# CODEJIN/multi_speaker_tts

Hardware: AMD Instinct MI355X
Metric: mel-frames/sec (train step) at batch 32x(128 tok,800 mel) (higher is better)
Workload: dtype f32

## Files before the change

multi_speaker_tts_amd/csrc/gemm.hip:

```cpp
#include "common.h"
#include <type_traits>
#include <cmath>
#include <cstdlib>

namespace mstts {

typedef float f32x16 __attribute__((ext_vector_type(16)));

constexpr int BK = 32;
constexpr int BN = 128;

struct GemmArgs {
    const float* A; const float* B; float* C; const float* bias;
    int M, N, K;
    long lda, ldb, ldc;
    int win_T, win_C, win_pad, win_dil;
    int act, accumulate, split_k;
    long stride_a, stride_b, stride_c;
    float alpha;
    int k_per_split;
    int body, tail_s, tail_kps;
    int band;
};

// ... 143 lines not shown
        for (int i = 0; i < NV; ++i)
            *reinterpret_cast<float4*>(s + (kr + i * KR) * ldS + c4 * 4) = reg[i];
    }
};

template <int WM, int WN>
__device__ __forceinline__ void gemm_store_tile(const GemmArgs& g, const f32x16 (&acc)[WM][WN], float* __restrict__ C, int row0, int col0,
                                                int lane, bool with_bias, bool atomic) {
#pragma unroll
    for (int i = 0; i < WM; ++i)
#pragma unroll
        for (int j = 0; j < WN; ++j) {
            const int col = col0 + j * 32 + (lane & 31);
            if (col >= g.N) continue;
            const float bv = (g.bias != nullptr && with_bias) ? g.bias[col] : 0.f;
#pragma unroll
            for (int r = 0; r < 16; ++r) {
                const int row = row0 + i * 32 + (r & 3) + 8 * (r >> 2) + 4 * (lane >> 5);
                if (row >= g.M) continue;
                float v = g.alpha * acc[i][j][r] + bv;
                float* dst = C + (long)row * g.ldc + col;
                if (atomic) {
                    atomicAdd(dst, v);
                } else {
                    v = apply_act(v, g.act);
                    if (g.accumulate) v += *dst;
                    *dst = v;
                }
            }
        }
}

template <int BM, bool TA, bool TB, bool VEC>
__global__ __launch_bounds__(256) void gemm_kernel(GemmArgs g) {
    constexpr int LDA_S = TA ? BM + 4 : BM + 2, LDB_S = TB ? BN + 2 : BN + 4;
    constexpr int A_FLOATS = (BK * LDA_S + 3) / 4 * 4;
    __shared__ __attribute__((aligned(16))) float smem[A_FLOATS + BK * LDB_S];
    float* As = smem;
    float* Bs = smem + A_FLOATS;

    const int tiles_n = (g.N + BN - 1) / BN;
    int tile = blockIdx.x, piece = -1;
    if (tile < g.body) {
        const int nb = g.body, q = nb >> 3, r = nb & 7, xcd = tile & 7, idx = tile >> 3;
        if (nb >= 64) tile = xcd * q + (xcd < r ? xcd : r) + idx;
    } else {
        const int u = tile - g.body;
        tile = g.body + u / g.tail_s;
        piece = u % g.tail_s;
    }
    const int tile_m = tile / tiles_n, tile_n = tile % tiles_n;
    const int batch = blockIdx.z / g.split_k, split = blockIdx.z % g.split_k;
    const float* A = g.A + (long)batch * g.stride_a;
    const float* B = g.B + (long)batch * g.stride_b;
    float* C = g.C + (long)batch * g.stride_c;
    const int m0 = tile_m * BM, n0 = tile_n * BN;
    const int kbeg = piece >= 0 ? piece * g.tail_kps : split * g.k_per_split;
    const int kend = min(g.K, kbeg + (piece >= 0 ? g.tail_kps : g.k_per_split));

    using LA = typename std::conditional<TA, LoaderMC<BM, VEC>, LoaderKC<BM, VEC>>::type;
    using LB = typename std::conditional<TB, LoaderKC<BN, VEC>, LoaderMC<BN, VEC>>::type;
    LA la; LB lb;

    const int lane = threadIdx.x & 63, wave = threadIdx.x >> 6;
    constexpr int WM = (BM >= 64) ? 2 : 1;
    constexpr int WN = (BM == 128) ? 2 : 1;
    const int wm = (BM == 128) ? (wave >> 1) : 0;
    const int wn = (BM == 128) ? (wave & 1) : wave;
    const int wrow = wm * WM * 32, wcol = wn * WN * 32;

    f32x16 acc[WM][WN];
#pragma unroll
    for (int i = 0; i < WM; ++i)
#pragma unroll
        for (int j = 0; j < WN; ++j)
#pragma unroll
            for (int r = 0; r < 16; ++r) acc[i][j][r] = 0.f;

    auto load_a = [&](int k) {
        if constexpr (TA) la.load(k, kend, g.lda, g.win_T);
        else la.load(k, kend, g.win_T, g.win_C, g.win_pad, g.win_dil);
    };
    auto load_b = [&](int k) {
        if constexpr (TB) lb.load(k, kend, 0, 1, 0, 1);
        else lb.load(k, kend, g.ldb, 0);
    };
    la.prepare(A, g.lda, m0, kbeg, g.M, g.win_T, g.win_C, g.win_pad, g.win_dil);
    lb.prepare(B, g.ldb, n0, kbeg, g.N, 0, 1, 0, 1);
    if (kbeg < kend) {
        load_a(kbeg);
        load_b(kbeg);
    }
    for (int k0 = kbeg; k0 < kend; k0 += BK) {
        __syncthreads();
        la.store(As, LDA_S);
        lb.store(Bs, LDB_S);
        __syncthreads();
        if (k0 + BK < kend) {
            load_a(k0 + BK);
            load_b(k0 + BK);
        }
        const int kh = lane >> 5, l31 = lane & 31;
        float a[2][WM], b[2][WN];
#pragma unroll
        for (int i = 0; i < WM; ++i) a[0][i] = As[kh * LDA_S + wrow + i * 32 + l31];
#pragma unroll
        for (int j = 0; j < WN; ++j) b[0][j] = Bs[kh * LDB_S + wcol + j * 32 + l31];
#pragma unroll
        for (int kk = 0; kk < BK; kk += 2) {
            const int cur = (kk >> 1) & 1, nxt = cur ^ 1;
            if (kk + 2 < BK) {
#pragma unroll
                for (int i = 0; i < WM; ++i) a[nxt][i] = As[(kk + 2 + kh) * LDA_S + wrow + i * 32 + l31];
#pragma unroll
                for (int j = 0; j < WN; ++j) b[nxt][j] = Bs[(kk + 2 + kh) * LDB_S + wcol + j * 32 + l31];
            }
            __builtin_amdgcn_sched_barrier(0);
#pragma unroll
            for (int i = 0; i < WM; ++i)
#pragma unroll
                for (int j = 0; j < WN; ++j)
                    acc[i][j] = __builtin_amdgcn_mfma_f32_32x32x2f32(a[cur][i], b[cur][j], acc[i][j], 0, 0, 0);
            __builtin_amdgcn_sched_barrier(0);
        }
    }

    gemm_store_tile<WM, WN>(g, acc, C, m0 + wrow, n0 + wcol, lane, split == 0 && piece <= 0, g.split_k > 1 || piece >= 0);
}

__global__ void gemm_tail_act_kernel(float* __restrict__ C, long ldc, int N, long n, int act) {
    const long i = (long)blockIdx.x * 256 + threadIdx.x;
    if (i >= n) return;
    float* p = C + (i / N) * ldc + (i % N);
    *p = apply_act(*p, act);
}

template <int BM, bool TA, bool TB>
static void launch_gemm(const GemmArgs& g, bool vec, dim3 grid, hipStream_t st) {
    if (vec) hipLaunchKernelGGL((gemm_kernel<BM, TA, TB, true>), grid, dim3(256), 0, st, g);
    else     hipLaunchKernelGGL((gemm_kernel<BM, TA, TB, false>), grid, dim3(256), 0, st, g);
}

#include "gemm_split.inc"

}

using namespace mstts;

static int g_tail_split = 1;
extern "C" int mstts_gemm_tail_split(int32_t on) { g_tail_split = on != 0; return MSTTS_OK; }
static int g_split3 = 1;
extern "C" int mstts_gemm_split3(int32_t on) { g_split3 = on != 0; return MSTTS_OK; }
static int g_split_big = 1;
extern "C" int mstts_gemm_split_big(int32_t on) { g_split_big = on != 0; return MSTTS_OK; }
static int g_split_big_min = 160;
namespace mstts { void gemm_bf16_set_big_min(int n); }
extern "C" int mstts_gemm_big_min_workgroups(int32_t f32_split, int32_t bf16) {
    if (f32_split > 0) g_split_big_min = f32_split;
    gemm_bf16_set_big_min(bf16);
    return MSTTS_OK;
}
static thread_local int t_deterministic = 0;
extern "C" int mstts_gemm_deterministic(int32_t on) { t_deterministic = on != 0; return MSTTS_OK; }
namespace mstts { int gemm_deterministic_now() { return t_deterministic; } }

extern "C" int mstts_gemm_f32(const mstts_gemm_desc* d, mstts_stream_t stream) {
    MSTTS_REQUIRE(d != nullptr, MSTTS_ERR_SHAPE, "gemm: null descriptor");
    MSTTS_REQUIRE(d->M >= 0 && d->N >= 0 && d->K >= 0, MSTTS_ERR_SHAPE, "gemm: negative dims");
    if (d->M == 0 || d->N == 0) return MSTTS_OK;
    MSTTS_REQUIRE(d->A && d->B && d->C, MSTTS_ERR_SHAPE, "gemm: null operand");
    MSTTS_REQUIRE(d->M < (1LL << 31) && d->N < (1LL << 31) && d->K < (1LL << 31), MSTTS_ERR_SHAPE, "gemm: dims exceed int32");
    MSTTS_REQUIRE(d->lda >= 0 && d->ldb >= 0 && d->lda < (1 << 24) && d->ldb < (1 << 24), MSTTS_ERR_SHAPE,
                  "gemm: row strides must be below 2^24 elements (tile-relative offsets are 32-bit)");
    const int batch = d->batch > 0 ? (int)d->batch : 1;
    int split = d->split_k > 1 ? d->split_k : 1;
    MSTTS_REQUIRE(split == 1 || (d->act == MSTTS_ACT_NONE), MSTTS_ERR_SHAPE,
                  "gemm: split_k needs act=none (output must be pre-zeroed or accumulated into)");
    if (d->win_T > 0) {
        MSTTS_REQUIRE(d->win_C > 0 && d->lda == d->win_C, MSTTS_ERR_SHAPE, "gemm: window mode needs lda == win_C");
        MSTTS_REQUIRE(d->win_C % 4 == 0, MSTTS_ERR_SHAPE, "gemm: window mode needs win_C %% 4 == 0");
    }
    GemmArgs g;
    g.A = d->A; g.B = d->B; g.C = d->C; g.bias = d->bias;
    g.M = (int)d->M; g.N = (int)d->N; g.K = (int)d->K;
    g.lda = d->lda; g.ldb = d->ldb; g.ldc = d->ldc;
    g.win_T = d->win_T; g.win_C = d->win_C > 0 ? d->win_C : 1; g.win_pad = d->win_pad; g.win_dil = d->win_dil > 0 ? d->win_dil : 1;
    g.act = d->act; g.accumulate = d->accumulate; g.split_k = split;
    g.stride_a = d->stride_a; g.stride_b = d->stride_b; g.stride_c = d->stride_c;
    g.alpha = d->alpha;
    int kps = ((g.K + split - 1) / split + BK - 1) / BK * BK;
    if (kps < BK) kps = BK;
    g.k_per_split = kps;
    bool vec = aligned16(d->A) && aligned16(d->B) && (d->lda % 4 == 0) && (d->ldb % 4 == 0) &&
               (d->stride_a % 4 == 0) && (d->stride_b % 4 == 0);
    vec = vec && (d->trans_a ? (d->M % 4 == 0) : (d->K % 4 == 0));
    vec = vec && (d->trans_b ? (d->K % 4 == 0) : (d->N % 4 == 0));
    if (d->win_T > 0) vec = vec && (d->win_C % 4 == 0);
    const bool skinny = d->M <= 32;
    int bm = skinny ? 32 : 128, tail_s = 1, tail_rem = 0;
    const bool split3 = g_split3 && !skinny && d->K >= 160 && (d->win_T <= 0 || (d->win_T >= BK && d->win_C >= BK)) && gemm_split_lds_ready();
    if (!skinny) {
        const double t128 = (double)cdiv(d->M, 128) * cdiv(d->N, BN) * batch * split, t64 = (double)cdiv(d->M, 64) * cdiv(d->N, BN) * batch * split;
        const double e128 = t128 / (ceil(t128 / 256.0) * 256.0), e64 = t64 / (ceil(t64 / 256.0) * 256.0);
        if (e64 * 0.95 > e128 && !split3) bm = 64;
        if (g_tail_split && !t_deterministic && batch == 1 && split == 1 && (d->act == MSTTS_ACT_NONE || !d->accumulate)) {
            double best = (bm == 128 ? ceil(t128 / 256.0) : ceil(t64 / 256.0) * 0.54);
            const int ktiles = cdiv(d->K, BK);
            for (int cand = 128; cand >= (split3 ? 128 : 64); cand -= 64) {
                const long t = (long)cdiv(d->M, cand) * cdiv(d->N, BN);
                int rem = (int)(t % 256);
                if (d->act != MSTTS_ACT_NONE) rem = (int)(t - (t - rem) / cdiv(d->N, BN) * cdiv(d->N, BN));
                if (split3 && t <= 128) rem = (int)t;
                else if (t <= 256 || rem == 0 || rem > 128) continue;
                int s = 256 / rem;
                if (s > 16) s = 16;
                if (s > ktiles / 8) s = ktiles / 8;
                if (s < 2) continue;
                const double c = ((double)(t / 256) + 1.25 / s + 0.06) * (cand == 128 ? 1.0 : 0.54);
                if (c < best) { best = c; bm = cand; tail_s = s; tail_rem = rem; }
            }
        }
    }
    hipStream_t st = (hipStream_t)stream;
    {
        const long big_wgs = (long)cdiv(d->M, GSB_BM) * cdiv(d->N, GSB_BN) * batch * split;
        if (split3 && g_split_big && d->M >= 192 && d->N >= 192 && big_wgs >= g_split_big_min && d->lda < (1 << 22) && d->ldb < (1 << 22) &&
            (d->win_T <= 0 || (d->win_T >= GSB_BK && d->win_C >= GSB_BK)) && (d->act == MSTTS_ACT_NONE || split == 1) && gemm_split_big_ready()) {
            int kpsb = ((g.K + split - 1) / split + GSB_BK - 1) / GSB_BK * GSB_BK;
            if (kpsb < GSB_BK) kpsb = GSB_BK;
            g.k_per_split = kpsb;
            g.body = 0; g.tail_s = 1; g.tail_kps = kpsb; g.band = 0;
            dim3 gridb(cdiv(d->M, GSB_BM) * cdiv(d->N, GSB_BN), 1, batch * split);
            const bool ta_ = d->trans_a != 0, tb_ = d->trans_b != 0;
            if (!ta_ && !tb_) launch_gemm_split_big<false, false>(g, vec, gridb, st);
            else if (!ta_ && tb_) launch_gemm_split_big<false, true>(g, vec, gridb, st);
            else if (ta_ && !tb_) launch_gemm_split_big<true, false>(g, vec, gridb, st);
            else launch_gemm_split_big<true, true>(g, vec, gridb, st);
            MSTTS_CHECK_LAUNCH("gemm_f32 (split, 256 x 256 tile)");
            return MSTTS_OK;
        }
    }
    const int tiles = cdiv(d->M, bm) * cdiv(d->N, BN);
    g.body = tiles; g.tail_s = 1; g.tail_kps = kps;
    g.band = (split3 && tail_s == 1 && cdiv(d->N, BN) > 8) ? 8 : 0;
    if (tail_s > 1) {
        const int rem = tail_rem, tiles_n = cdiv(d->N, BN);
        g.body = tiles - rem; g.tail_s = tail_s;
        g.tail_kps = (cdiv(g.K, BK) + tail_s - 1) / tail_s * BK;
        if (!d->accumulate) {
            const long r0 = (long)(g.body / tiles_n) * bm;
            if (hipMemset2DAsync(d->C + r0 * d->ldc, (size_t)d->ldc * 4, 0, (size_t)d->N * 4, (size_t)(d->M - r0), st) != hipSuccess)
                MSTTS_REQUIRE(false, MSTTS_ERR_LAUNCH, "gemm: clearing the tail tiles failed");
        }
    }
    dim3 grid(g.body + (tiles - g.body) * g.tail_s, 1, batch * split);
    const bool ta = d->trans_a != 0, tb = d->trans_b != 0;
    if (split3) {
        if (!ta && !tb) launch_gemm_split<false, false>(g, vec, grid, st);
        else if (!ta && tb) launch_gemm_split<false, true>(g, vec, grid, st);
        else if (ta && !tb) launch_gemm_split<true, false>(g, vec, grid, st);
        else launch_gemm_split<true, true>(g, vec, grid, st);
    } else if (skinny) {
        if (!ta && !tb) launch_gemm<32, false, false>(g, vec, grid, st);
        else if (!ta && tb) launch_gemm<32, false, true>(g, vec, grid, st);
        else if (ta && !tb) launch_gemm<32, true, false>(g, vec, grid, st);
        else launch_gemm<32, true, true>(g, vec, grid, st);
    } else if (bm == 64) {
        if (!ta && !tb) launch_gemm<64, false, false>(g, vec, grid, st);
        else if (!ta && tb) launch_gemm<64, false, true>(g, vec, grid, st);
        else if (ta && !tb) launch_gemm<64, true, false>(g, vec, grid, st);
        else launch_gemm<64, true, true>(g, vec, grid, st);
    } else {
        if (!ta && !tb) launch_gemm<128, false, false>(g, vec, grid, st);
        else if (!ta && tb) launch_gemm<128, false, true>(g, vec, grid, st);
        else if (ta && !tb) launch_gemm<128, true, false>(g, vec, grid, st);
        else launch_gemm<128, true, true>(g, vec, grid, st);
    }
    MSTTS_CHECK_LAUNCH("gemm_f32");
    if (tail_s > 1 && d->act != MSTTS_ACT_NONE) {
        const long r0 = (long)(g.body / cdiv(d->N, BN)) * bm;
        const long n = (d->M - r0) * d->N;
        hipLaunchKernelGGL(gemm_tail_act_kernel, dim3((unsigned)cdiv(n, 256)), dim3(256), 0, st, d->C + r0 * d->ldc, d->ldc, (int)d->N, n, d->act);
        MSTTS_CHECK_LAUNCH("gemm_f32 tail activation");
    }
    return MSTTS_OK;
}
```

multi_speaker_tts_amd/csrc/gemm_split.inc:

```

typedef __bf16 gs_bf16x8 __attribute__((ext_vector_type(8)));
typedef __bf16 gs_bf16x4 __attribute__((ext_vector_type(4)));
constexpr int GS_BM = 128, GS_LD = 40;
constexpr int GS_PLANE = 128 * GS_LD;

struct Split3 { gs_bf16x4 hi, mid, lo; };
__device__ __forceinline__ uint32_t gs_cvt_pk(float a, float b) {
    uint32_t r;
    asm("v_cvt_pk_bf16_f32 %0, %1, %2" : "=v"(r) : "v"(a), "v"(b));
    return r;
}
__device__ __forceinline__ float gs_sub(float a, uint32_t b_bits) {
    float r;
    asm("v_sub_f32 %0, %1, %2" : "=v"(r) : "v"(a), "v"(b_bits));
    return r;
}
__device__ __forceinline__ void gs_split2(float x0, float x1, uint32_t& hi, uint32_t& mid, uint32_t& lo) {
    hi = gs_cvt_pk(x0, x1);
    x0 = gs_sub(x0, hi << 16); x1 = gs_sub(x1, hi & 0xffff0000u);
    mid = gs_cvt_pk(x0, x1);
    x0 = gs_sub(x0, mid << 16); x1 = gs_sub(x1, mid & 0xffff0000u);
    lo = gs_cvt_pk(x0, x1);
}
__device__ __forceinline__ Split3 gs_split4(float a, float b, float c, float d) {
// ... 200 lines not shown
        using LA = typename std::conditional<TA, GsLoaderMC<VEC, WIN>, GsLoaderKC<VEC, WIN>>::type;
        using LB = typename std::conditional<TB, GsLoaderKC<VEC, false>, GsLoaderMC<VEC, false>>::type;
        if (wave < 8) {
            const int tid = threadIdx.x - 256;
            LA la;
            la.prepare(tid, g.A + (long)batch * g.stride_a, g.lda, m0, kbeg, g.M, g.win_T, g.win_C, g.win_pad, g.win_dil);
            gs_produce([&](float4 (&r)[4], int k) {
                           if constexpr (TA) la.load(tid, r, k, kend, g.lda, g.win_T);
                           else la.load(tid, r, k, kend, g.win_T, g.win_C, g.win_pad, g.win_dil);
                       },
                       [&](const float4 (&r)[4], __bf16* dst) { la.store(tid, r, dst); }, gs_lds, kbeg, nt2);
        } else {
            const int tid = threadIdx.x - 512;
            LB lb;
            lb.prepare(tid, g.B + (long)batch * g.stride_b, g.ldb, n0, kbeg, g.N, 0, 1, 0, 1);
            gs_produce([&](float4 (&r)[4], int k) {
                           if constexpr (TB) lb.load(tid, r, k, kend, 0, 1, 0, 1);
                           else lb.load(tid, r, k, kend, g.ldb, 0);
                       },
                       [&](const float4 (&r)[4], __bf16* dst) { lb.store(tid, r, dst); }, gs_lds + 3 * GS_PLANE, kbeg, nt2);
        }
        return;
    }

    float* C = g.C + (long)batch * g.stride_c;
    const int lane = threadIdx.x & 63;
    const int wrow = (wave >> 1) * 64, wcol = (wave & 1) * 64;
    const int l31 = lane & 31, kg = lane >> 5;

    f32x16 acc[2][2];
#pragma unroll
    for (int i = 0; i < 2; ++i)
#pragma unroll
        for (int j = 0; j < 2; ++j)
#pragma unroll
            for (int r = 0; r < 16; ++r) acc[i][j][r] = 0.f;

    const int aoff = (wrow + l31) * GS_LD + kg * 8, boff = 3 * GS_PLANE + (wcol + l31) * GS_LD + kg * 8;
    gs_bf16x8 fa[2][2][3], fb[2][2][3];
    auto frags = [&](int set, const __bf16* buf, int ks) {
#pragma unroll
        for (int p = 0; p < 3; ++p) {
#pragma unroll
            for (int i = 0; i < 2; ++i) fa[set][i][p] = *reinterpret_cast<const gs_bf16x8*>(buf + aoff + p * GS_PLANE + i * 32 * GS_LD + ks * 16);
#pragma unroll
            for (int j = 0; j < 2; ++j) fb[set][j][p] = *reinterpret_cast<const gs_bf16x8*>(buf + boff + p * GS_PLANE + j * 32 * GS_LD + ks * 16);
        }
    };
    auto products = [&](int set) {
#pragma unroll
        for (int tt = 0; tt < GS_NPROD; ++tt) {
            const int pa = (tt == 0) ? 0 : (tt == 1) ? 1 : (tt == 2) ? 0 : (tt == 3) ? 1 : (tt == 4) ? 2 : 0;
            const int pb = (tt == 0) ? 0 : (tt == 1) ? 0 : (tt == 2) ? 1 : (tt == 3) ? 1 : (tt == 4) ? 0 : 2;
#pragma unroll
            for (int i = 0; i < 2; ++i)
#pragma unroll
                for (int j = 0; j < 2; ++j)
                    acc[i][j] = __builtin_amdgcn_mfma_f32_32x32x16_bf16(fa[set][i][pa], fb[set][j][pb], acc[i][j], 0, 0, 0);
        }
    };
    GS_BAR(0);
    frags(0, gs_lds, 0);
    for (int t = 0; t < nt2; ++t) {
        const __bf16* buf = gs_lds + (t & 1) * GS_BUF;
        frags(1, buf, 1);
        __builtin_amdgcn_sched_barrier(0);
        products(0);
        __builtin_amdgcn_sched_barrier(0);
        GS_BAR(0);
        frags(0, gs_lds + ((t + 1) & 1) * GS_BUF, 0);
        __builtin_amdgcn_sched_barrier(0);
        products(1);
        __builtin_amdgcn_sched_barrier(0);
    }
#ifdef GS_STAMP
    if (stamp && (threadIdx.x & 63) == 0) { unsigned long long* o = (unsigned long long*)g.bias; o[0] = acc_wait; o[1] = __builtin_readcyclecounter() - t_begin; o[2] = nt2; o[3] = wall_clock64() - w_begin; }
    if (stamp) return;
#endif
    gemm_store_tile<2, 2>(g, acc, C, m0 + wrow, n0 + wcol, lane, split == 0 && piece <= 0, g.split_k > 1 || piece >= 0);
}

constexpr int GSB_BM = 256, GSB_BN = 256, GSB_BK = 16, GSB_LD = 24, GSB_THREADS = 512;
constexpr int GSB_PLANE = 256 * GSB_LD;
constexpr int GSB_BUF = 6 * GSB_PLANE;
constexpr size_t GSB_LDS_BYTES = 2 * GSB_BUF * sizeof(__bf16);
__device__ __forceinline__ void gsb_put(__bf16* __restrict__ p, const Split3& s) {
    *reinterpret_cast<gs_bf16x4*>(p) = s.hi;
    *reinterpret_cast<gs_bf16x4*>(p + GSB_PLANE) = s.mid;
    *reinterpret_cast<gs_bf16x4*>(p + 2 * GSB_PLANE) = s.lo;
}
template <bool VEC, bool WIN>
struct GsbLoaderKC {
    static constexpr int NV = 2;
    const float* ubase;
    unsigned voff[2], rmask;
    int t_row[2], tap, kc, ld_;
    __device__ __forceinline__ bool mine(int) const { return true; }
    __device__ __forceinline__ void prepare(int tid, const float* __restrict__ base, long ld, int row0, int k0, int rows, int wT, int wC, int wpad, int wdil) {
        const int k4 = tid & 3, r = tid >> 2;
        rmask = 0; ld_ = (int)ld;
#pragma unroll
        for (int i = 0; i < 2; ++i) {
            const int row = row0 + r + i * 128;
            if (row < rows) rmask |= 1u << i;
            voff[i] = (unsigned)((r + i * 128) * (int)ld) + (WIN ? 0u : (unsigned)(k4 * 4));
            if (WIN) t_row[i] = row % wT;
        }
        if (WIN) {
            const int k = k0 + k4 * 4;
            tap = k / wC; kc = k - tap * wC;
            ubase = base + ((long)row0 - (long)wpad * wdil) * ld;
        } else {
            ubase = base + (long)row0 * ld + k0;
        }
    }
    __device__ __forceinline__ void load(int tid, float4 (&reg)[4], int k0, int kmax, long, int wT, int wC, int wpad, int wdil) {
        const int k4 = tid & 3;
        const int k = k0 + k4 * 4;
        const bool kok = k < kmax;
        const int sh = WIN ? (tap - wpad) * wdil : 0;
        const unsigned wadd = WIN ? (unsigned)(tap * wdil * ld_ + kc) : 0u;
#pragma unroll
        for (int i = 0; i < 2; ++i) {
            float4 v = make_float4(0.f, 0.f, 0.f, 0.f);
            bool ok = kok && ((rmask >> i) & 1u);
            if (WIN) {
                const int t = t_row[i] + sh;
                ok = ok && t >= 0 && t < wT;
            }
            if (VEC) {
                v = gemm_ld4(ok ? ubase + (voff[i] + wadd) : gemm_zero16);
            } else if (ok) {
                const float* p = ubase + (voff[i] + wadd);
                v.x = p[0];
                if (k + 1 < kmax) v.y = p[1];
                if (k + 2 < kmax) v.z = p[2];
                if (k + 3 < kmax) v.w = p[3];
            }
            reg[i] = v;
        }
        if (WIN) {
            kc += GSB_BK;
            const bool wrap = kc >= wC;
            kc -= wrap ? wC : 0; tap += wrap ? 1 : 0;
        } else {
            ubase += GSB_BK;
        }
    }
    __device__ __forceinline__ void store(int tid, const float4 (&reg)[4], __bf16* __restrict__ s) const {
        const int k4 = tid & 3, r = tid >> 2;
#pragma unroll
        for (int i = 0; i < 2; ++i) gsb_put(s + (r + i * 128) * GSB_LD + k4 * 4, gs_split4(reg[i].x, reg[i].y, reg[i].z, reg[i].w));
    }
};
template <bool VEC, bool WIN, int HALF>
struct GsbLoaderMC {
    const float* ubase;
    unsigned voff[4];
    int sh, t_k[4], cols_left;
    __device__ __forceinline__ bool mine(int tid) const { return (tid >> 8) == HALF; }
    __device__ __forceinline__ void prepare(int tid, const float* __restrict__ base, long ld, int col0, int k0, int cols, int wT, int wC, int wpad, int wdil) {
        const int u = tid & 255, kq = u & 3, c4 = u >> 2;
        const int col = col0 + c4 * 4;
        cols_left = cols - col;
        if (WIN) {
            const int tp = col / wC, cm = col - tp * wC;
            sh = (tp - wpad) * wdil;
#pragma unroll
            for (int i = 0; i < 4; ++i) {
                t_k[i] = (k0 + kq * 4 + i) % wT;
                voff[i] = (unsigned)((kq * 4 + i + tp * wdil) * (int)ld + cm);
            }
            ubase = base + ((long)k0 - (long)wpad * wdil) * ld;
        } else {
            sh = 0;
#pragma unroll
            for (int i = 0; i < 4; ++i) voff[i] = (unsigned)((kq * 4 + i) * (int)ld + c4 * 4);
            ubase = base + (long)k0 * ld + col0;
        }
    }
    __device__ __forceinline__ void load(int tid, float4 (&reg)[4], int k0, int kmax, long ld, int wT, int, int, int) {
        const int kq = tid & 3;
#pragma unroll
        for (int i = 0; i < 4; ++i) {
            const int k = k0 + kq * 4 + i;
            float4 v = make_float4(0.f, 0.f, 0.f, 0.f);
            bool ok = k < kmax && cols_left > 0;
            if (WIN) {
                const int t = t_k[i] + sh;
                ok = ok && t >= 0 && t < wT;
                t_k[i] += GSB_BK;
                t_k[i] -= (t_k[i] >= wT) ? wT : 0;
            }
            if (VEC) {
                v = gemm_ld4(ok ? ubase + voff[i] : gemm_zero16);
            } else if (ok) {
                const float* p = ubase + voff[i];
                v.x = p[0];
                if (cols_left > 1) v.y = p[1];
                if (cols_left > 2) v.z = p[2];
                if (cols_left > 3) v.w = p[3];
            }
            reg[i] = v;
        }
        ubase += GSB_BK * ld;
    }
    __device__ __forceinline__ void store(int tid, const float4 (&reg)[4], __bf16* __restrict__ s) const {
        const int u = tid & 255, kq = u & 3, c4 = u >> 2;
        __bf16* p = s + (c4 * 4) * GSB_LD + kq * 4;
        gsb_put(p, gs_split4(reg[0].x, reg[1].x, reg[2].x, reg[3].x));
        gsb_put(p + GSB_LD, gs_split4(reg[0].y, reg[1].y, reg[2].y, reg[3].y));
        gsb_put(p + 2 * GSB_LD, gs_split4(reg[0].z, reg[1].z, reg[2].z, reg[3].z));
        gsb_put(p + 3 * GSB_LD, gs_split4(reg[0].w, reg[1].w, reg[2].w, reg[3].w));
    }
};

template <bool TA, bool TB, bool VEC, bool WIN>
__global__ __launch_bounds__(GSB_THREADS) void gemm_split_big_kernel(GemmArgs g) {
    extern __shared__ __attribute__((aligned(16))) __bf16 gs_lds[];
    const int tiles_n = (g.N + GSB_BN - 1) / GSB_BN;
    int tile = blockIdx.x;
    {
        const int nb = gridDim.x, q = nb >> 3, r = nb & 7, xcd = tile & 7, idx = tile >> 3;
        if (nb >= 64) tile = xcd * q + (xcd < r ? xcd : r) + idx;
    }
    const int tile_m = tile / tiles_n, tile_n = tile % tiles_n;
    const int batch = blockIdx.z / g.split_k, split = blockIdx.z % g.split_k;
    float* C = g.C + (long)batch * g.stride_c;
    const int m0 = tile_m * GSB_BM, n0 = tile_n * GSB_BN;
    const int kbeg = split * g.k_per_split;
    const int kend = min(g.K, kbeg + g.k_per_split);
    const int nt = kend > kbeg ? (kend - kbeg + GSB_BK - 1) / GSB_BK : 0;
    const int tid = threadIdx.x, lane = tid & 63, wave = __builtin_amdgcn_readfirstlane(tid >> 6);
    const int wrow = (wave >> 2) * 128, wcol = (wave & 3) * 64;
    const int l31 = lane & 31, kg = lane >> 5;

    using LA = typename std::conditional<TA, GsbLoaderMC<VEC, WIN, 0>, GsbLoaderKC<VEC, WIN>>::type;
    using LB = typename std::conditional<TB, GsbLoaderKC<VEC, false>, GsbLoaderMC<VEC, false, 1>>::type;
    LA la; LB lb;
    const bool a_mine = la.mine(tid), b_mine = lb.mine(tid);
    if (a_mine) la.prepare(tid, g.A + (long)batch * g.stride_a, g.lda, m0, kbeg, g.M, g.win_T, g.win_C, g.win_pad, g.win_dil);
    if (b_mine) lb.prepare(tid, g.B + (long)batch * g.stride_b, g.ldb, n0, kbeg, g.N, 0, 1, 0, 1);
    float4 ra[4], rb[4];
    auto load = [&](int k) {
        if (a_mine) la.load(tid, ra, k, kend, g.lda, g.win_T, g.win_C, g.win_pad, g.win_dil);
        if (b_mine) lb.load(tid, rb, k, kend, g.ldb, 0, 1, 0, 1);
    };
    auto store = [&](int buf) {
        if (a_mine) la.store(tid, ra, gs_lds + buf * GSB_BUF);
        if (b_mine) lb.store(tid, rb, gs_lds + buf * GSB_BUF + 3 * GSB_PLANE);
    };

    f32x16 acc[4][2];
#pragma unroll
    for (int i = 0; i < 4; ++i)
#pragma unroll
        for (int j = 0; j < 2; ++j)
#pragma unroll
            for (int r = 0; r < 16; ++r) acc[i][j][r] = 0.f;

    const int aoff = (wrow + l31) * GSB_LD + kg * 8, boff = 3 * GSB_PLANE + (wcol + l31) * GSB_LD + kg * 8;
    gs_bf16x8 fb[2][3], fa0[4], fa1[4];
    auto ldA = [&](gs_bf16x8 (&f)[4], const __bf16* buf, int p) {
#pragma unroll
        for (int i = 0; i < 4; ++i) f[i] = *reinterpret_cast<const gs_bf16x8*>(buf + aoff + p * GSB_PLANE + i * 32 * GSB_LD);
    };
    auto ldB = [&](const __bf16* buf) {
#pragma unroll
        for (int p = 0; p < 3; ++p)
#pragma unroll
            for (int j = 0; j < 2; ++j) fb[j][p] = *reinterpret_cast<const gs_bf16x8*>(buf + boff + p * GSB_PLANE + j * 32 * GSB_LD);
    };
    auto mm = [&](const gs_bf16x8 (&f)[4], int pb) {
#pragma unroll
        for (int i = 0; i < 4; ++i)
#pragma unroll
            for (int j = 0; j < 2; ++j)
                acc[i][j] = __builtin_amdgcn_mfma_f32_32x32x16_bf16(f[i], fb[j][pb], acc[i][j], 0, 0, 0);
    };

    if (nt > 0) {
        load(kbeg);
        store(0);
        load(kbeg + GSB_BK);
        gs_barrier();
        for (int t = 0; t < nt; ++t) {
            const __bf16* buf = gs_lds + (t & 1) * GSB_BUF;
            ldB(buf); ldA(fa0, buf, 0); ldA(fa1, buf, 1);
            mm(fa0, 0); mm(fa0, 1); mm(fa0, 2);
            ldA(fa0, buf, 2);
            store((t + 1) & 1);
            load(kbeg + (t + 2) * GSB_BK);
            mm(fa1, 0); mm(fa1, 1);
            mm(fa0, 0);
            gs_barrier();
        }
    }
    gemm_store_tile<4, 2>(g, acc, C, m0 + wrow, n0 + wcol, lane, split == 0, g.split_k > 1);
}

static int gemm_split_big_ready() {
    static int memo[64];
    int dev = 0;
    if (hipGetDevice(&dev) != hipSuccess || dev < 0 || dev >= 64) return 0;
    if (!memo[dev]) {
        bool ok = true;
#define GSB_ATTR1(TA_, TB_, V_, W_) ok = ok && hipFuncSetAttribute((const void*)gemm_split_big_kernel<TA_, TB_, V_, W_>, hipFuncAttributeMaxDynamicSharedMemorySize, (int)GSB_LDS_BYTES) == hipSuccess
#define GSB_ATTR(TA_, TB_) GSB_ATTR1(TA_, TB_, true, true); GSB_ATTR1(TA_, TB_, true, false); GSB_ATTR1(TA_, TB_, false, true); GSB_ATTR1(TA_, TB_, false, false)
        GSB_ATTR(false, false); GSB_ATTR(false, true); GSB_ATTR(true, false); GSB_ATTR(true, true);
#undef GSB_ATTR
#undef GSB_ATTR1
        if (!ok) (void)hipGetLastError();
        memo[dev] = ok ? 2 : 1;
    }
    return memo[dev] == 2;
}

template <bool TA, bool TB>
static void launch_gemm_split_big(const GemmArgs& g, bool vec, dim3 grid, hipStream_t st) {
    const bool win = g.win_T > 0;
    if (vec && win)  hipLaunchKernelGGL((gemm_split_big_kernel<TA, TB, true, true>), grid, dim3(GSB_THREADS), GSB_LDS_BYTES, st, g);
    else if (vec)    hipLaunchKernelGGL((gemm_split_big_kernel<TA, TB, true, false>), grid, dim3(GSB_THREADS), GSB_LDS_BYTES, st, g);
    else if (win)    hipLaunchKernelGGL((gemm_split_big_kernel<TA, TB, false, true>), grid, dim3(GSB_THREADS), GSB_LDS_BYTES, st, g);
    else             hipLaunchKernelGGL((gemm_split_big_kernel<TA, TB, false, false>), grid, dim3(GSB_THREADS), GSB_LDS_BYTES, st, g);
}

static int gemm_split_lds_ready() {
    static int memo[64];
    int dev = 0;
    if (hipGetDevice(&dev) != hipSuccess || dev < 0 || dev >= 64) return 0;
    if (!memo[dev]) {
        bool ok = true;
#define GS_ATTR1(TA_, TB_, V_, W_) ok = ok && hipFuncSetAttribute((const void*)gemm_split_kernel<TA_, TB_, V_, W_>, hipFuncAttributeMaxDynamicSharedMemorySize, (int)GS_LDS_BYTES) == hipSuccess
#define GS_ATTR(TA_, TB_) GS_ATTR1(TA_, TB_, true, true); GS_ATTR1(TA_, TB_, true, false); GS_ATTR1(TA_, TB_, false, true); GS_ATTR1(TA_, TB_, false, false)
        GS_ATTR(false, false); GS_ATTR(false, true); GS_ATTR(true, false); GS_ATTR(true, true);
#undef GS_ATTR
#undef GS_ATTR1
        if (!ok) (void)hipGetLastError();
        memo[dev] = ok ? 2 : 1;
    }
    return memo[dev] == 2;
}

template <bool TA, bool TB>
static void launch_gemm_split(const GemmArgs& g, bool vec, dim3 grid, hipStream_t st) {
    const bool win = g.win_T > 0;
    if (vec && win)  hipLaunchKernelGGL((gemm_split_kernel<TA, TB, true, true>), grid, dim3(GS_THREADS), GS_LDS_BYTES, st, g);
    else if (vec)    hipLaunchKernelGGL((gemm_split_kernel<TA, TB, true, false>), grid, dim3(GS_THREADS), GS_LDS_BYTES, st, g);
    else if (win)    hipLaunchKernelGGL((gemm_split_kernel<TA, TB, false, true>), grid, dim3(GS_THREADS), GS_LDS_BYTES, st, g);
    else             hipLaunchKernelGGL((gemm_split_kernel<TA, TB, false, false>), grid, dim3(GS_THREADS), GS_LDS_BYTES, st, g);
}
```

multi_speaker_tts_amd/lib.py:

```python
from __future__ import annotations

import ctypes as C
import os

import torch

_HERE = os.path.dirname(os.path.abspath(__file__))
LIB_PATH = os.path.join(_HERE, "libmstts_hip.so")

ACT_NONE, ACT_RELU, ACT_TANH, ACT_SIGMOID = 0, 1, 2, 3

vp, i64, i32, f32, u64, u32 = C.c_void_p, C.c_int64, C.c_int32, C.c_float, C.c_uint64, C.c_uint32


class GemmDesc(C.Structure):
    _fields_ = [("A", vp), ("B", vp), ("C", vp), ("bias", vp),
                ("M", i64), ("N", i64), ("K", i64), ("lda", i64), ("ldb", i64), ("ldc", i64),
                ("trans_a", i32), ("trans_b", i32), ("win_T", i32), ("win_C", i32), ("win_pad", i32),
                ("act", i32), ("accumulate", i32), ("split_k", i32),
                ("batch", i64), ("stride_a", i64), ("stride_b", i64), ("stride_c", i64), ("alpha", f32), ("win_dil", i32)]


class LstmPointFwd(C.Structure):
    _fields_ = [("B", i64), ("H", i64), ("gates_h", vp), ("gates_parts", i32), ("gates_pstride", i64), ("xw", vp), ("xw_sb", i64), ("xw_st", i64), ("bias", vp),
# ... 141 lines not shown
    "mstts_lsa_proj_pack_floats": (i64, []),
    "mstts_lsa_proj_pack": (i32, [vp, i64, i64, i64, vp, vp]),
    "mstts_lsa_step_qp_ws_bytes": (i64, [i64, i64]),
    "mstts_lsa_step_prenet_supported": (i32, [i64, i64]),
    "mstts_lsa_step_fwd_qp": (i32, [P(LsaConst), vp, i64, vp, i64, vp, vp, vp, i64, i64, vp, vp, vp, vp, vp, vp, i64, vp, i64, P(CellPackedDst),
                                    P(LsaPrenet), vp, C.c_uint32, i32, vp]),
    "mstts_lsa_step_fwd_q": (i32, [P(LsaConst), vp, i64, vp, i64, i32, vp, vp, vp, vp, vp, i64, vp, i64, P(CellPackedDst), vp, C.c_uint32, i32, vp]),
    "mstts_lsa_step_fwd_selftest": (i32, [P(LsaConst), vp, i32, i64, vp, vp, vp, vp, vp, i64, vp, C.c_uint32, i32, vp]),
    "mstts_lsa_dalign_bwd": (i32, [P(LsaConst), vp, i64, vp, i64, i32, i64, vp, vp, vp, vp, vp]),
    "mstts_lsa_denergy_bwd": (i32, [P(LsaConst), vp, vp, vp, vp, vp, vp, vp, vp]),
    "mstts_lsa_param_bwd": (i32, [P(LsaConst), i64, vp, vp, vp, vp, vp, vp, vp, vp, vp]),
    "mstts_lsa_param_bwd_ws_floats": (i64, [i64, i64, i64]),
    "mstts_lsa_fold_location": (i32, [vp, vp, vp, vp, vp, i64, i64, i64, vp]),
    "mstts_lsa_filter_by_unit": (i32, [vp, vp, i64, i64, vp]),
    "mstts_lsa_unfold_location_grad": (i32, [vp, vp, vp, vp, vp, vp, vp, vp, i64, i64, i64, vp]),
    "mstts_tts_loss_fwd_bwd": (i32, [vp, vp, vp, vp, vp, i64, i64, i64, i32, f32, vp, vp, vp, vp, vp]),
    "mstts_l2_loss_acc": (i32, [vp, vp, i64, vp, vp]),
    "mstts_shift_frames": (i32, [vp, vp, i64, i64, i64, vp]),
    "mstts_unpack_proj": (i32, [vp, i64, vp, vp, i64, i64, i64, vp]),
    "mstts_pack_dproj": (i32, [vp, vp, vp, i64, i64, i64, i64, vp]),
    "mstts_speaker_tile": (i32, [vp, vp, vp, i64, i64, i64, i64, i64, vp]),
    "mstts_conv_kernel_flip": (i32, [vp, vp, i64, i64, i64, vp]),
    "mstts_transpose01": (i32, [vp, vp, i64, i64, i64, vp]),
    "mstts_speaker_finalize": (i32, [vp, vp, i64, i64, i64, i64, vp]),
    "mstts_adam_tf": (i32, [vp, vp, vp, vp, vp, f32, f32, f32, f32, f32, f32, i64, vp]),
    "mstts_stft_mel": (i32, [vp, i64, f32, vp, vp, i32, i32, i32, i32, f32, vp, vp, i64, vp]),
    "mstts_stft_mel_ws_floats": (i64, [i64, i32, i64]),
    "mstts_stft_fft_supported": (i32, [i32, i32]),
    "mstts_stft_fft": (i32, [vp, vp, vp, i32, f32, vp, vp, vp, vp, i32, i32, i32, i32, f32, f32, vp, vp, i64, vp, vp, f32, i32, vp]),
    "mstts_fold_rows": (i32, [vp, vp, i64, i64, i64, i64, vp]),
    "mstts_decoder_bf16_splits": (i32, [i64, i64, i64, P(i32)]),
    "mstts_skinny_bf16_fwd_splits": (i32, [i64, i64]),
    "mstts_skinny_bf16_bwd_splits": (i32, [i64, i64]),
    "mstts_pack_bf16_fwd": (i32, [vp, i64, vp, i64, i64, i32, vp]),
    "mstts_pack_bf16_bwd": (i32, [vp, i64, vp, i64, i64, i32, vp]),
    "mstts_skinny_fwd_bf16": (i32, [vp, i64, vp, vp, i64, i64, i64, i64, i32, vp]),
    "mstts_skinny_bwd_bf16": (i32, [vp, i64, vp, vp, i64, i64, i64, i64, i32, vp]),
    "mstts_ge2e_ws_floats": (i64, [i64, i64, i64]),
    "mstts_ge2e_loss_fwd_bwd": (i32, [vp, i64, i64, i64, i64, vp, vp, vp, i64, vp, vp]),
    "mstts_wg_overlap_add": (i32, [vp, vp, vp, i64, i64, i64, i64, i64, vp]),
    "mstts_wg_gate": (i32, [vp, i64, vp, i64, i64, vp]),
    "mstts_wg_gate_add": (i32, [vp, i64, vp, vp, i64, i64, vp]),
    "mstts_wg_res_skip": (i32, [vp, vp, vp, vp, i64, i64, i32, i32, vp]),
    "mstts_wg_coupling_inv": (i32, [vp, vp, vp, vp, f32, vp, i64, i64, i64, vp]),
    "mstts_philox_normal": (i32, [vp, i64, u64, u32, f32, vp]),
    "mstts_wg_weight_norm_fwd": (i32, [vp, i64, i64, vp]),
    "mstts_wg_weight_norm_bwd": (i32, [vp, i64, i64, vp]),
    "mstts_wg_coupling_fwd": (i32, [vp, vp, vp, vp, i64, i64, i64, vp, i64, i64, vp]),
    "mstts_wg_coupling_bwd": (i32, [vp, vp, vp, i64, i64, i64, vp, f32, vp, vp, i64, i64, vp]),
    "mstts_wg_inv1x1_logdet": (i32, [vp, vp, vp, i64, f32, vp, vp]),
    "mstts_wg_gate_bwd": (i32, [vp, i64, vp, vp, vp, i64, i64, i64, vp]),
    "mstts_wg_res_skip_bwd": (i32, [vp, vp, vp, vp, i64, i64, i32, vp]),
    "mstts_wg_overlap_add_bwd": (i32, [vp, vp, i64, i64, i64, i64, i64, i64, vp]),
    "mstts_wg_bias_fold": (i32, [vp, vp, vp, i64, i64, vp]),
    "mstts_adam_tf_clip": (i32, [vp, vp, vp, vp, vp, f32, f32, f32, f32, f32, f32, i64, vp]),
    "mstts_lstm_seq_fwd": (i32, [P(LstmSeqFwd), vp]),
    "mstts_lstm_seq_bwd": (i32, [P(LstmSeqBwd), vp]),
    "mstts_lstm_seq_fwd_pair": (i32, [P(LstmSeqFwd), P(LstmSeqFwd), vp]),
    "mstts_lstm_seq_bwd_pair": (i32, [P(LstmSeqBwd), P(LstmSeqBwd), vp]),
    "mstts_persist_lstm_supported": (i32, [i64, i64]),
    "mstts_persist_lstm_pack_floats": (i64, []),
    "mstts_persist_lstm_ws_bytes": (i64, []),
    "mstts_persist_lstm_pack": (i32, [vp, i64, vp, vp, vp]),
    "mstts_persist_lstm_supported_n": (i32, [i64, i64, i32]),
    "mstts_persist_lstm_fwd_supported_n": (i32, [i64, i64, i32]),
    "mstts_persist_lstm_pack_fwd": (i32, [vp, i64, i64, vp, vp]),
    "mstts_persist_lstm_ws_bytes_n": (i64, [i64, i32]),
    "mstts_persist_lstm_hist_floats_n": (i64, [i64, i64, i32]),
    "mstts_persist_lstm_bwd_floats_n": (i64, [i64, i64, i32]),
    "mstts_lstm_seq_fwd_persistent": (i32, [P(LstmSeqFwd), vp, vp, vp, vp, vp]),
    "mstts_lstm_seq_bwd_persistent": (i32, [P(LstmSeqBwd), vp, vp, vp, vp, vp, vp]),
    "mstts_persist_lstm_hist_floats": (i64, [i64]),
    "mstts_persist_lstm_bwd_floats": (i64, [i64]),
    "mstts_lstm_seq_fwd_pair_persistent": (i32, [P(LstmSeqFwd), P(LstmSeqFwd), vp, vp, vp, vp, vp, vp]),
    "mstts_lstm_seq_bwd_pair_persistent": (i32, [P(LstmSeqBwd), P(LstmSeqBwd), vp, vp, vp, vp, vp, vp, vp]),
    "mstts_lstm_point_bwd_pair": (i32, [P(LstmPointBwd), P(LstmPointBwd), vp]),
    "mstts_skinny_bwd_pair": (i32, [vp, vp, i64, vp, vp, i64, vp, vp, i64, i64, i64, i64, i32, vp]),
    "mstts_lstm_seq_ws_floats": (i64, [i64, i64, i32]),
    "mstts_decoder_train_fwd": (i32, [P(DecoderTrain), vp]),
    "mstts_decoder_train_bwd": (i32, [P(DecoderTrainBwd), vp]),
    "mstts_persist_fwd_supported": (i32, [i64, i64, i64, i64, i64, i64]),
    "mstts_persist_fwd_ws_bytes": (i64, []),
    "mstts_persist_pack_floats": (i64, [i32]),
    "mstts_persist_pack": (i32, [vp, vp, vp, vp, vp, vp, vp, vp]),
    "mstts_decoder_train_fwd_persistent": (i32, [P(DecoderTrain), P(PersistDesc), vp]),
    "mstts_persist_opk_floats": (i64, [i64]),
    "mstts_persist_unpack_history": (i32, [vp, P(DecoderTrain), vp]),
    "mstts_persist_bwd_supported": (i32, [i64, i64, i64, i64, i64, i64]),
    "mstts_persist_bwd_ws_bytes": (i64, []),
    "mstts_persist_bwd_pack_floats": (i64, [i32]),
    "mstts_persist_bwd_pack": (i32, [vp, vp, vp, vp, vp, vp, vp]),
    "mstts_decoder_train_bwd_persistent": (i32, [P(DecoderTrainBwd), P(PersistDesc), vp]),
    "mstts_decoder_train_bwd_ws_floats": (i64, [i64, i64, i64, i64, i64, i64]),
    "mstts_decoder_train_bwd_parts": (i32, [i64, i64]),
    "mstts_decoder_train_ws_floats": (i32, [i64, i64, i64, i64, C.POINTER(i64), C.POINTER(i64)]),
    "mstts_skinny_fwd_splits": (i32, [i64, i64]),
    "mstts_skinny_fwd": (i32, [vp, i64, vp, i64, vp, i64, i64, i64, i64, i32, vp]),
    "mstts_skinny_bwd_splits": (i32, [i64, i64]),
    "mstts_skinny_bwd": (i32, [vp, i64, vp, i64, vp, i64, i64, i64, i64, i32, vp]),
    "mstts_pack_skinny_bwd": (i32, [vp, i64, vp, i64, i64, i32, vp]),
    "mstts_skinny_bwd_packed": (i32, [vp, i64, vp, vp, i64, i64, i64, i64, i32, vp]),
    "mstts_decoder_infer_fast": (i32, [i64, i64, i64, i64, i64, i64]),
    "mstts_decoder_infer_steps": (i32, [P(DecoderInfer), i64, i64, vp]),
    "mstts_persist_infer_supported": (i32, [i64, i64, i64, i64, i64, i64, i64, i64]),
    "mstts_persist_infer_ws_bytes": (i64, []),
    "mstts_persist_infer_pack_floats": (i64, []),
    "mstts_persist_infer_pack": (i32, [vp, vp, i64, vp, vp, vp]),
    "mstts_decoder_infer_persistent": (i32, [P(DecoderInfer), P(PersistInferDesc), vp]),
    "mstts_decoder_infer_ws_floats": (i64, [i64, i64, i64, i64, i64, i64]),
    "mstts_f32_to_bf16": (i32, [vp, vp, i64, vp]),
    "mstts_bf16_to_f32": (i32, [vp, vp, i64, vp]),
    "mstts_bf16_chunks_sum": (i32, [vp, i32, i64, i64, vp, vp]),
    "mstts_probe_begin": (i32, [i32, i64]),
    "mstts_probe_result": (i64, [C.POINTER(C.c_double), C.POINTER(C.c_double)]),
}

_lib = None


ABI_VERSION = 5


class MsttsError(RuntimeError):
    pass


def load():
    global _lib
    if _lib is not None:
        return _lib
    from . import build as _b
    if _b.needs_build():
        try:
            _b.build()
        except RuntimeError as e:
            if "hipcc not found" in str(e) and os.path.exists(LIB_PATH) and not os.path.exists(LIB_PATH + ".hash"):
                import warnings
                warnings.warn("libmstts_hip.so could not be checked against its sources (hipcc not found); loading the existing library")
            else:
                raise
    lib = C.CDLL(LIB_PATH)
    for name, (res, args) in SIGNATURES.items():
        fn = getattr(lib, name)
        fn.restype = res
        fn.argtypes = args
    if lib.mstts_abi_version() != ABI_VERSION:
        raise MsttsError("libmstts_hip.so reports ABI version %d, this binding is written for %d: rebuild the library (python -m multi_speaker_tts_amd.build --force)"
                         % (lib.mstts_abi_version(), ABI_VERSION))
    env = os.environ.get
    if env("MSTTS_GEMM_SPLIT3", "1") == "0":
        lib.mstts_gemm_split3(0)
    if env("MSTTS_GEMM_SPLIT_BIG", "1") == "0":
        lib.mstts_gemm_split_big(0)
    if env("MSTTS_GEMM_BF16_BIG", "1") == "0":
        lib.mstts_gemm_bf16_big(0)
    if env("MSTTS_GEMM_BF16_AUTOCUT", "1") == "0":
        lib.mstts_gemm_bf16_autocut(0)
    if env("MSTTS_GEMM_SPLIT_BIG_MIN") or env("MSTTS_GEMM_BF16_BIG_MIN"):
        lib.mstts_gemm_big_min_workgroups(int(env("MSTTS_GEMM_SPLIT_BIG_MIN", "0")), int(env("MSTTS_GEMM_BF16_BIG_MIN", "0")))
    _lib = lib
    return lib


class deterministic_gemm:
    _depth = __import__("threading").local()

    def __enter__(self):
        n = getattr(self._depth, "n", 0)
        if n == 0:
            load().mstts_gemm_deterministic(1)
        self._depth.n = n + 1
        return self

    def __exit__(self, *exc):
        self._depth.n -= 1
        if self._depth.n == 0:
            load().mstts_gemm_deterministic(0)
        return False

    def __call__(self, fn):
        import functools

        @functools.wraps(fn)
        def wrapped(*a, **k):
            with deterministic_gemm():
                return fn(*a, **k)
        return wrapped


_raw_stream = getattr(torch._C, "_cuda_getCurrentRawStream", None)


def stream():
    if _raw_stream is not None:
        return C.c_void_p(_raw_stream(torch.cuda.current_device()))
    return C.c_void_p(torch.cuda.current_stream().cuda_stream)


def ptr(t, offset=0):
    if t is None:
        return None
    return t.data_ptr() + offset * t.element_size()


def call(name, *args):
    lib = load()
    rc = getattr(lib, name)(*args, stream())
    if rc != 0:
        raise MsttsError("%s failed (%d): %s" % (name, rc, lib.mstts_last_error().decode()))


def gemm(A, B, Cm, M, N, K, lda, ldb, ldc, bias=None, trans_a=False, trans_b=False, act=ACT_NONE, accumulate=False,
         split_k=1, win=None, batch=1, strides=(0, 0, 0), alpha=1.0, a_off=0, b_off=0, c_off=0, bias_off=0, bf16=False):
    d = GemmDesc()
    d.A, d.B, d.C, d.bias = ptr(A, a_off), ptr(B, b_off), ptr(Cm, c_off), ptr(bias, bias_off)
    d.M, d.N, d.K, d.lda, d.ldb, d.ldc = M, N, K, lda, ldb, ldc
    d.trans_a, d.trans_b = int(trans_a), int(trans_b)
    if win is not None:
        d.win_T, d.win_C, d.win_pad = win[:3]
        d.win_dil = win[3] if len(win) > 3 else 1
    d.act, d.accumulate, d.split_k = act, int(accumulate), split_k
    d.batch, d.stride_a, d.stride_b, d.stride_c = batch, strides[0], strides[1], strides[2]
    d.alpha = alpha
    call("mstts_gemm_bf16" if bf16 else "mstts_gemm_f32", C.byref(d))
```

Baseline: 626,700.

## Interleave LDS staging stores with MFMA phases in split-big GEMM main loop

Adds a PIPE variant of the 256x256 split-bf16 GEMM kernel for non-windowed operands. It breaks the next tile's register-to-LDS split/store into per-unit slots, interleaves them with the MFMA groups and the next global load, and fences each phase with sched_barriers. The aim is to hide the bf16 three-way split conversion and LDS write latency behind matrix math instead of running them as a separate serial phase. It is on by default, and MSTTS_GEMM_SPLIT_BIG=2 falls back to the old loop. It doubles the kernel template instantiations and may raise register pressure.

```diff
diff --git a/multi_speaker_tts_amd/csrc/gemm.hip b/multi_speaker_tts_amd/csrc/gemm.hip
--- a/multi_speaker_tts_amd/csrc/gemm.hip
+++ b/multi_speaker_tts_amd/csrc/gemm.hip
@@ -319,7 +319,7 @@
 static int g_split3 = 1;
 extern "C" int mstts_gemm_split3(int32_t on) { g_split3 = on != 0; return MSTTS_OK; }
 static int g_split_big = 1;
-extern "C" int mstts_gemm_split_big(int32_t on) { g_split_big = on != 0; return MSTTS_OK; }
+extern "C" int mstts_gemm_split_big(int32_t on) { g_split_big = on == 2 ? 2 : on != 0; return MSTTS_OK; }
 static int g_split_big_min = 160;
 namespace mstts { void gemm_bf16_set_big_min(int n); }
 extern "C" int mstts_gemm_big_min_workgroups(int32_t f32_split, int32_t bf16) {
@@ -398,11 +398,11 @@
             g.k_per_split = kpsb;
             g.body = 0; g.tail_s = 1; g.tail_kps = kpsb; g.band = 0;
             dim3 gridb(cdiv(d->M, GSB_BM) * cdiv(d->N, GSB_BN), 1, batch * split);
-            const bool ta_ = d->trans_a != 0, tb_ = d->trans_b != 0;
-            if (!ta_ && !tb_) launch_gemm_split_big<false, false>(g, vec, gridb, st);
-            else if (!ta_ && tb_) launch_gemm_split_big<false, true>(g, vec, gridb, st);
-            else if (ta_ && !tb_) launch_gemm_split_big<true, false>(g, vec, gridb, st);
-            else launch_gemm_split_big<true, true>(g, vec, gridb, st);
+            const bool ta_ = d->trans_a != 0, tb_ = d->trans_b != 0, pipe = g_split_big != 2 && d->win_T <= 0;
+            if (!ta_ && !tb_) launch_gemm_split_big<false, false>(g, vec, pipe, gridb, st);
+            else if (!ta_ && tb_) launch_gemm_split_big<false, true>(g, vec, pipe, gridb, st);
+            else if (ta_ && !tb_) launch_gemm_split_big<true, false>(g, vec, pipe, gridb, st);
+            else launch_gemm_split_big<true, true>(g, vec, pipe, gridb, st);
             MSTTS_CHECK_LAUNCH("gemm_f32 (split, 256 x 256 tile)");
             return MSTTS_OK;
         }
diff --git a/multi_speaker_tts_amd/csrc/gemm_split.inc b/multi_speaker_tts_amd/csrc/gemm_split.inc
--- a/multi_speaker_tts_amd/csrc/gemm_split.inc
+++ b/multi_speaker_tts_amd/csrc/gemm_split.inc
@@ -376,6 +376,12 @@
 #pragma unroll
         for (int i = 0; i < 2; ++i) gsb_put(s + (r + i * 128) * GSB_LD + k4 * 4, gs_split4(reg[i].x, reg[i].y, reg[i].z, reg[i].w));
     }
+    static constexpr int NU = 2;
+    template <int U>
+    __device__ __forceinline__ void store_unit(int tid, const float4 (&reg)[4], __bf16* __restrict__ s) const {
+        const int k4 = tid & 3, r = tid >> 2;
+        gsb_put(s + (r + U * 128) * GSB_LD + k4 * 4, gs_split4(reg[U].x, reg[U].y, reg[U].z, reg[U].w));
+    }
 };
 template <bool VEC, bool WIN, int HALF>
 struct GsbLoaderMC {
@@ -437,9 +443,19 @@
         gsb_put(p + 2 * GSB_LD, gs_split4(reg[0].z, reg[1].z, reg[2].z, reg[3].z));
         gsb_put(p + 3 * GSB_LD, gs_split4(reg[0].w, reg[1].w, reg[2].w, reg[3].w));
     }
+    static constexpr int NU = 4;
+    template <int U>
+    __device__ __forceinline__ void store_unit(int tid, const float4 (&reg)[4], __bf16* __restrict__ s) const {
+        const int u = tid & 255, kq = u & 3, c4 = u >> 2;
+        __bf16* p = s + (c4 * 4 + U) * GSB_LD + kq * 4;
+        if constexpr (U == 0) gsb_put(p, gs_split4(reg[0].x, reg[1].x, reg[2].x, reg[3].x));
+        if constexpr (U == 1) gsb_put(p, gs_split4(reg[0].y, reg[1].y, reg[2].y, reg[3].y));
+        if constexpr (U == 2) gsb_put(p, gs_split4(reg[0].z, reg[1].z, reg[2].z, reg[3].z));
+        if constexpr (U == 3) gsb_put(p, gs_split4(reg[0].w, reg[1].w, reg[2].w, reg[3].w));
+    }
 };
 
-template <bool TA, bool TB, bool VEC, bool WIN>
+template <bool TA, bool TB, bool VEC, bool WIN, bool PIPE>
 __global__ __launch_bounds__(GSB_THREADS) void gemm_split_big_kernel(GemmArgs g) {
     extern __shared__ __attribute__((aligned(16))) __bf16 gs_lds[];
     const int tiles_n = (g.N + GSB_BN - 1) / GSB_BN;
@@ -503,7 +519,59 @@
                 acc[i][j] = __builtin_amdgcn_mfma_f32_32x32x16_bf16(f[i], fb[j][pb], acc[i][j], 0, 0, 0);
     };
 
-    if (nt > 0) {
+    auto slot = [&](auto S, int buf) {
+        constexpr int u = decltype(S)::value;
+        __bf16* dst = gs_lds + buf * GSB_BUF;
+        if constexpr (u < LA::NU) { if (a_mine) la.template store_unit<u>(tid, ra, dst); }
+        if constexpr (u < LB::NU) { if (b_mine) lb.template store_unit<u>(tid, rb, dst + 3 * GSB_PLANE); }
+    };
+    using S0 = std::integral_constant<int, 0>; using S1 = std::integral_constant<int, 1>;
+    using S2 = std::integral_constant<int, 2>; using S3 = std::integral_constant<int, 3>;
+    static_assert(LA::NU <= 4 && LB::NU <= 4, "four staging slots");
+
+    if (PIPE && nt > 0) {
+        load(kbeg);
+        store(0);
+        load(kbeg + GSB_BK);
+        gs_barrier();
+        for (int t = 0; t < nt; ++t) {
+            const __bf16* buf = gs_lds + (t & 1) * GSB_BUF;
+            const int nb = (t + 1) & 1;
+#pragma unroll
+            for (int j = 0; j < 2; ++j) fb[j][0] = *reinterpret_cast<const gs_bf16x8*>(buf + boff + j * 32 * GSB_LD);
+            ldA(fa0, buf, 0);
+#pragma unroll
+            for (int p = 1; p < 3; ++p)
+#pragma unroll
+                for (int j = 0; j < 2; ++j) fb[j][p] = *reinterpret_cast<const gs_bf16x8*>(buf + boff + p * GSB_PLANE + j * 32 * GSB_LD);
+            __builtin_amdgcn_sched_barrier(0);
+            slot(S0{}, nb);
+            __builtin_amdgcn_sched_barrier(0);
+            mm(fa0, 0);
+            __builtin_amdgcn_sched_barrier(0);
+            ldA(fa1, buf, 1);
+            slot(S1{}, nb);
+            __builtin_amdgcn_sched_barrier(0);
+            mm(fa0, 1);
+            __builtin_amdgcn_sched_barrier(0);
+            slot(S2{}, nb);
+            __builtin_amdgcn_sched_barrier(0);
+            mm(fa0, 2);
+            __builtin_amdgcn_sched_barrier(0);
+            ldA(fa0, buf, 2);
+            slot(S3{}, nb);
+            __builtin_amdgcn_sched_barrier(0);
+            mm(fa1, 0);
+            __builtin_amdgcn_sched_barrier(0);
+            load(kbeg + (t + 2) * GSB_BK);
+            __builtin_amdgcn_sched_barrier(0);
+            mm(fa1, 1);
+            __builtin_amdgcn_sched_barrier(0);
+            mm(fa0, 0);
+            __builtin_amdgcn_sched_barrier(0);
+            gs_barrier();
+        }
+    } else if (nt > 0) {
         load(kbeg);
         store(0);
         load(kbeg + GSB_BK);
@@ -529,24 +597,31 @@
     if (hipGetDevice(&dev) != hipSuccess || dev < 0 || dev >= 64) return 0;
     if (!memo[dev]) {
         bool ok = true;
-#define GSB_ATTR1(TA_, TB_, V_, W_) ok = ok && hipFuncSetAttribute((const void*)gemm_split_big_kernel<TA_, TB_, V_, W_>, hipFuncAttributeMaxDynamicSharedMemorySize, (int)GSB_LDS_BYTES) == hipSuccess
+#define GSB_ATTR2(TA_, TB_, V_, W_, P_) ok = ok && hipFuncSetAttribute((const void*)gemm_split_big_kernel<TA_, TB_, V_, W_, P_>, hipFuncAttributeMaxDynamicSharedMemorySize, (int)GSB_LDS_BYTES) == hipSuccess
+#define GSB_ATTR1(TA_, TB_, V_, W_) GSB_ATTR2(TA_, TB_, V_, W_, true); GSB_ATTR2(TA_, TB_, V_, W_, false)
 #define GSB_ATTR(TA_, TB_) GSB_ATTR1(TA_, TB_, true, true); GSB_ATTR1(TA_, TB_, true, false); GSB_ATTR1(TA_, TB_, false, true); GSB_ATTR1(TA_, TB_, false, false)
         GSB_ATTR(false, false); GSB_ATTR(false, true); GSB_ATTR(true, false); GSB_ATTR(true, true);
 #undef GSB_ATTR
 #undef GSB_ATTR1
+#undef GSB_ATTR2
         if (!ok) (void)hipGetLastError();
         memo[dev] = ok ? 2 : 1;
     }
     return memo[dev] == 2;
 }
 
+template <bool TA, bool TB, bool P>
+static void launch_gemm_split_big_loop(const GemmArgs& g, bool vec, dim3 grid, hipStream_t st) {
+    const bool win = g.win_T > 0;
+    if (vec && win)  hipLaunchKernelGGL((gemm_split_big_kernel<TA, TB, true, true, P>), grid, dim3(GSB_THREADS), GSB_LDS_BYTES, st, g);
+    else if (vec)    hipLaunchKernelGGL((gemm_split_big_kernel<TA, TB, true, false, P>), grid, dim3(GSB_THREADS), GSB_LDS_BYTES, st, g);
+    else if (win)    hipLaunchKernelGGL((gemm_split_big_kernel<TA, TB, false, true, P>), grid, dim3(GSB_THREADS), GSB_LDS_BYTES, st, g);
+    else             hipLaunchKernelGGL((gemm_split_big_kernel<TA, TB, false, false, P>), grid, dim3(GSB_THREADS), GSB_LDS_BYTES, st, g);
+}
 template <bool TA, bool TB>
-static void launch_gemm_split_big(const GemmArgs& g, bool vec, dim3 grid, hipStream_t st) {
-    const bool win = g.win_T > 0;
-    if (vec && win)  hipLaunchKernelGGL((gemm_split_big_kernel<TA, TB, true, true>), grid, dim3(GSB_THREADS), GSB_LDS_BYTES, st, g);
-    else if (vec)    hipLaunchKernelGGL((gemm_split_big_kernel<TA, TB, true, false>), grid, dim3(GSB_THREADS), GSB_LDS_BYTES, st, g);
-    else if (win)    hipLaunchKernelGGL((gemm_split_big_kernel<TA, TB, false, true>), grid, dim3(GSB_THREADS), GSB_LDS_BYTES, st, g);
-    else             hipLaunchKernelGGL((gemm_split_big_kernel<TA, TB, false, false>), grid, dim3(GSB_THREADS), GSB_LDS_BYTES, st, g);
+static void launch_gemm_split_big(const GemmArgs& g, bool vec, bool pipe, dim3 grid, hipStream_t st) {
+    if (pipe) launch_gemm_split_big_loop<TA, TB, true>(g, vec, grid, st);
+    else launch_gemm_split_big_loop<TA, TB, false>(g, vec, grid, st);
 }
 
 static int gemm_split_lds_ready() {
diff --git a/multi_speaker_tts_amd/lib.py b/multi_speaker_tts_amd/lib.py
--- a/multi_speaker_tts_amd/lib.py
+++ b/multi_speaker_tts_amd/lib.py
@@ -317,6 +317,8 @@
         lib.mstts_gemm_split3(0)
     if env("MSTTS_GEMM_SPLIT_BIG", "1") == "0":
         lib.mstts_gemm_split_big(0)
+    elif env("MSTTS_GEMM_SPLIT_BIG", "1") == "2":
+        lib.mstts_gemm_split_big(2)
     if env("MSTTS_GEMM_BF16_BIG", "1") == "0":
         lib.mstts_gemm_bf16_big(0)
     if env("MSTTS_GEMM_BF16_AUTOCUT", "1") == "0":
```

After: 628,400 (median of 6 runs). No clear change (+0.3%).
